# cc-ai/climategan

Hardware: AMD Instinct MI355X
Metric: 640x640 images/sec (G+D step): per-domain sample slots per second of the joint Masker+Painter training step (update_G + update_D), global batch 32 per domain (higher is better)
Workload: dtype bf16

## Files before the change

climategan_amd/csrc/conv3x3_lds.h:

```cpp
#pragma once
#include "cgan_common.h"

struct Conv3x3LdsArgs {
  const uint16_t* x;
  const u32x4* w;
  const float* bias;
  const uint16_t* res;
  uint16_t* y;
  int n, h, w_;
  int hi, wi;
  int pad, reflect;
  int hx, wx;
  int cin;
  int cin_s, cin_p, cout, cout_s, ctiles, ksteps;
  int in_ups, act, has_res, res_ups;
  float slope;
  int shuffle;
  int shuffle_w;
  int k, stride;
};

bool conv3x3_lds_applicable(const CganConvDesc* d);
int conv3x3_lds_launch(const Conv3x3LdsArgs& a, int dtype, hipStream_t s);
bool conv_smallcin_applicable(const CganConvDesc* d);
int conv_smallcin_launch(const Conv3x3LdsArgs& a, int dtype, hipStream_t s);
```

climategan_amd/csrc/conv3x3_lds.hip:

```cpp
#include "conv3x3_lds.h"

namespace {

constexpr int TW = 16, TH = 16, WAVES = 4, PT = TH / WAVES;
constexpr int HPW = TW + 2, HPH = TH + 2, HP = HPH * HPW;
constexpr int XDMA = (HP * 4 + 63) / 64;
constexpr int XBUF_BYTES = XDMA * 1024;
constexpr int MAX_NCT = 5;
CGAN_KNOB(int, g_lds_nct, 0);
CGAN_KNOB(int, g_c4_enabled, 1);

__device__ __forceinline__ int xq_addr(int q, int slot) { return q * 64 + ((slot ^ ((q >> 1) & 3)) << 4); }

__device__ __attribute__((aligned(16))) unsigned int g_zeros[64];

__device__ __forceinline__ void halo_coord(const Conv3x3LdsArgs& p, int& yy, int& xx) {
  if (p.reflect) {
    yy = yy < 0 ? -yy : yy;
    xx = xx < 0 ? -xx : xx;
    yy = yy >= p.hi ? 2 * p.hi - 2 - yy : yy;
    xx = xx >= p.wi ? 2 * p.wi - 2 - xx : xx;
  }
}

#define STAGE_BARRIER()                                            \
  do {                                                             \
    asm volatile("s_waitcnt vmcnt(0) lgkmcnt(0)" ::: "memory");    \
    __builtin_amdgcn_s_barrier();                                  \
    asm volatile("" ::: "memory");                                 \
  } while (0)

template <typename T, int NCT, bool RES = true>
__device__ __forceinline__ void conv3x3_epilogue(const Conv3x3LdsArgs& p, f32x4 (&acc)[NCT][PT], unsigned char* smem,
                                                 int n, int ty0, int tx0, int ct0, int wave, int j, int g) {
  if (p.shuffle) {
    const int a = g >> 1, b = g & 1;
#pragma unroll
    for (int t = 0; t < PT; ++t) {
      const int yy = ty0 + wave * PT + t, xx = tx0 + j;
      const int oy = 2 * yy + a, ox = 2 * xx + b;
      if (yy < p.h && xx < p.w_ && oy < p.shuffle && ox < p.shuffle_w && ct0 == 0) {
        const f32x4 v = acc[0][t];
        const u32x4 o = {pack2<T>(v[0], v[1]), pack2<T>(v[2], v[3]), 0u, 0u};
        *reinterpret_cast<u32x4*>(p.y + (((size_t)n * p.shuffle + oy) * p.shuffle_w + ox) * 8) = o;
      }
    }
    return;
  }
  __syncthreads();
  unsigned char* yt = smem;
  const bool pad_c = p.cout < p.cout_s;
  f32x4 bias_q[NCT];
#pragma unroll
  for (int c = 0; c < NCT; ++c) {
    const int ch = (ct0 + c) * 16 + g * 4;
    bias_q[c] = (p.bias && ch < p.cout_s) ? *reinterpret_cast<const f32x4*>(p.bias + ch) : (f32x4){0.f, 0.f, 0.f, 0.f};
  }
  u32x2 rq[RES ? PT : 1][RES ? NCT : 1];
  if (RES && p.has_res) {
#pragma unroll
    for (int t = 0; t < PT; ++t) {
      const int yy = ty0 + wave * PT + t, xx = tx0 + j;
      const bool pin = yy < p.h && xx < p.w_;
      size_t rbase = 0;
      if (pin) {
        if (p.res_ups) rbase = (((size_t)n * (p.h >> 1) + (yy >> 1)) * (p.w_ >> 1) + (xx >> 1)) * p.cout_s;
        else rbase = (((size_t)n * p.h + yy) * p.w_ + xx) * p.cout_s;
      }
#pragma unroll
      for (int c = 0; c < NCT; ++c) {
        const int ch = (ct0 + c) * 16 + g * 4;
        rq[t][c] = (u32x2){0u, 0u};
        if (pin && ch < p.cout_s) rq[t][c] = *reinterpret_cast<const u32x2*>(p.res + rbase + ch);
      }
    }
    __builtin_amdgcn_sched_barrier(0);
    __builtin_amdgcn_s_waitcnt(0x0F70);
  }
#pragma unroll
  for (int t = 0; t < PT; ++t) {
    const int row = wave * PT + t;
    const int yy = ty0 + row, xx = tx0 + j;
    const bool pin = yy < p.h && xx < p.w_;
#pragma unroll
    for (int c = 0; c < NCT; ++c) {
      const int ch = (ct0 + c) * 16 + g * 4;
      float v[4];
#pragma unroll
      for (int r = 0; r < 4; ++r) v[r] = acc[c][t][r];
      if (ch < p.cout_s) {
#pragma unroll
        for (int r = 0; r < 4; ++r) v[r] += bias_q[c][r];
        if (RES && p.has_res && pin) {
          const u32x2 rv = rq[RES ? t : 0][RES ? c : 0];
          float r0, r1, r2, r3;
          unpack2<T>(rv[0], r0, r1);
          unpack2<T>(rv[1], r2, r3);
          v[0] = cgan_res_apply(v[0], r0, p.has_res); v[1] = cgan_res_apply(v[1], r1, p.has_res);
          v[2] = cgan_res_apply(v[2], r2, p.has_res); v[3] = cgan_res_apply(v[3], r3, p.has_res);
        }
        act_apply_n(v, p.act, p.slope);
        if (pad_c) {
#pragma unroll
          for (int r = 0; r < 4; ++r)
            if (ch + r >= p.cout) v[r] = 0.f;
        }
      }
      u32x2 o;
      o[0] = pack2<T>(v[0], v[1]);
      o[1] = pack2<T>(v[2], v[3]);
      *reinterpret_cast<u32x2*>(yt + ((row * 16 + j) * NCT + c) * 32 + g * 8) = o;
    }
  }
  __syncthreads();
#pragma unroll
  for (int k = 0; k < 2 * NCT; ++k) {
    const int id = k * (WAVES * 64) + threadIdx.x;
    const int pix = id / (2 * NCT), cc = id - pix * (2 * NCT);
    const int yy = ty0 + (pix >> 4), xx = tx0 + (pix & 15);
    const int ch = ct0 * 16 + cc * 8;
    if (yy < p.h && xx < p.w_ && ch < p.cout_s)
      CGAN_ST_STREAM(*reinterpret_cast<const u32x4*>(yt + id * 16),
                     reinterpret_cast<u32x4*>(p.y + (((size_t)n * p.h + yy) * p.w_ + xx) * p.cout_s + ch));
  }
}

template <typename T, int NCT>
__global__ __launch_bounds__(WAVES * 64, 2) void conv3x3_lds_kernel(Conv3x3LdsArgs p) {
  const u32x4* zero_page = reinterpret_cast<const u32x4*>(g_zeros);
  constexpr int STAGE_BYTES = 3 * NCT * 1024;
  extern __shared__ __attribute__((aligned(16))) unsigned char smem[];
  unsigned char* xbuf = smem;
  unsigned char* wbuf = xbuf + 2 * XBUF_BYTES;

  const int lane = threadIdx.x & 63;
  const int wave = __builtin_amdgcn_readfirstlane(threadIdx.x >> 6);
  const int j = lane & 15;
  const int g = lane >> 4;

  const int tiles_x = (p.w_ + TW - 1) / TW, tiles_y = (p.h + TH - 1) / TH;
  int tile = blockIdx.x;
  const int txi = tile % tiles_x;
  tile /= tiles_x;
  const int tyi = tile % tiles_y;
  const int n = tile / tiles_y;
  const int ty0 = tyi * TH, tx0 = txi * TW;
  const int ct0 = blockIdx.y * NCT;
  const int nq = p.cin_p / 32;
  const int nstages = nq * 3;

  auto issue_x = [&](int q) {
    unsigned char* dst = xbuf + (q & 1) * XBUF_BYTES;
    for (int i = wave; i < XDMA; i += WAVES) {
      const int idx = i * 64 + lane;
      const int pix = idx >> 2, spos = idx & 3;
      const int slot = spos ^ ((pix >> 1) & 3);
      const int py = pix / HPW, px = pix - py * HPW;
      int yy = ty0 - p.pad + py, xx = tx0 - p.pad + px;
      halo_coord(p, yy, xx);
      const int ch = q * 32 + slot * 8;
      const u32x4* src = zero_page;
      if (pix < HP && yy >= 0 && yy < p.hi && xx >= 0 && xx < p.wi && ch < p.cin_s) {
        const int sy = p.in_ups ? (yy >> 1) : yy, sx = p.in_ups ? (xx >> 1) : xx;
        src = reinterpret_cast<const u32x4*>(p.x + (((size_t)n * p.hx + sy) * p.wx + sx) * p.cin_s + ch);
      }
      __builtin_amdgcn_global_load_lds((const __attribute__((address_space(1))) void*)src,
                                       (__attribute__((address_space(3))) void*)(dst + i * 1024), 16, 0, 0);
    }
  };
  auto issue_w = [&](int s) {
    const int q = s / 3, dx = s - q * 3;
    unsigned char* dst = wbuf + (s & 1) * STAGE_BYTES;
#pragma unroll
    for (int i0 = 0; i0 < 3 * NCT; i0 += WAVES) {
      const int i = i0 + wave;
      if (i < 3 * NCT) {
        const int dy = i / NCT, c = i - dy * NCT;
        const int ct = min(ct0 + c, p.ctiles - 1);
        const u32x4* src = p.w + ((size_t)ct * p.ksteps + (dy * 3 + dx) * nq + q) * 64 + lane;
        __builtin_amdgcn_global_load_lds((const __attribute__((address_space(1))) void*)src,
                                         (__attribute__((address_space(3))) void*)(dst + i * 1024), 16, 0, 0);
      }
    }
  };

  issue_x(0);
  issue_w(0);

  f32x4 acc[NCT][PT];
#pragma unroll
  for (int c = 0; c < NCT; ++c)
#pragma unroll
    for (int t = 0; t < PT; ++t) acc[c][t] = (f32x4){0.f, 0.f, 0.f, 0.f};

  for (int q = 0; q < nq; ++q) {
    const unsigned char* xb = xbuf + (q & 1) * XBUF_BYTES;
    for (int dx = 0; dx < 3; ++dx) {
      const int s = q * 3 + dx;
      STAGE_BARRIER();
      if (dx == 0 && q + 1 < nq) issue_x(q + 1);
      if (s + 1 < nstages) issue_w(s + 1);
      u32x4 bfr[PT + 2];
#pragma unroll
      for (int r = 0; r < PT + 2; ++r) {
        const int qq = (wave * PT + r) * HPW + (j + dx);
        bfr[r] = *reinterpret_cast<const u32x4*>(xb + xq_addr(qq, g));
      }
      const unsigned char* wb = wbuf + (s & 1) * STAGE_BYTES + lane * 16;
#pragma unroll
      for (int dy = 0; dy < 3; ++dy) {
        u32x4 a[NCT];
#pragma unroll
        for (int c = 0; c < NCT; ++c) a[c] = *reinterpret_cast<const u32x4*>(wb + (dy * NCT + c) * 1024);
#pragma unroll
        for (int c = 0; c < NCT; ++c)
#pragma unroll
          for (int t = 0; t < PT; ++t)
            acc[c][t] = mfma16(as_vec8<T>(a[c]), as_vec8<T>(bfr[t + dy]), acc[c][t]);
      }
    }
  }

  conv3x3_epilogue<T, NCT>(p, acc, smem, n, ty0, tx0, ct0, wave, j, g);
}

template <typename T, int NCT>
__global__ __launch_bounds__(WAVES * 64, 4) void conv3x3_lds_onechunk_kernel(Conv3x3LdsArgs p) {
  const u32x4* zero_page = reinterpret_cast<const u32x4*>(g_zeros);
  extern __shared__ __attribute__((aligned(16))) unsigned char smem[];
  unsigned char* xbuf = smem;
  unsigned char* wbuf = xbuf + XBUF_BYTES;

  const int lane = threadIdx.x & 63;
  const int wave = __builtin_amdgcn_readfirstlane(threadIdx.x >> 6);
  const int j = lane & 15;
  const int g = lane >> 4;
  const int tiles_x = (p.w_ + TW - 1) / TW, tiles_y = (p.h + TH - 1) / TH;
  int tile = blockIdx.x;
  const int txi = tile % tiles_x;
  tile /= tiles_x;
  const int tyi = tile % tiles_y;
  const int n = tile / tiles_y;
  const int ty0 = tyi * TH, tx0 = txi * TW;
  const int ct0 = blockIdx.y * NCT;

  for (int i = wave; i < XDMA; i += WAVES) {
    const int idx = i * 64 + lane;
    const int pix = idx >> 2, spos = idx & 3;
    const int slot = spos ^ ((pix >> 1) & 3);
    const int py = pix / HPW, px = pix - py * HPW;
    int yy = ty0 - p.pad + py, xx = tx0 - p.pad + px;
    halo_coord(p, yy, xx);
    const int ch = slot * 8;
    const u32x4* src = zero_page;
    if (pix < HP && yy >= 0 && yy < p.hi && xx >= 0 && xx < p.wi && ch < p.cin_s) {
      const int sy = p.in_ups ? (yy >> 1) : yy, sx = p.in_ups ? (xx >> 1) : xx;
      src = reinterpret_cast<const u32x4*>(p.x + (((size_t)n * p.hx + sy) * p.wx + sx) * p.cin_s + ch);
    }
    __builtin_amdgcn_global_load_lds((const __attribute__((address_space(1))) void*)src,
                                     (__attribute__((address_space(3))) void*)(xbuf + i * 1024), 16, 0, 0);
  }
#pragma unroll
  for (int i0 = 0; i0 < 9 * NCT; i0 += WAVES) {
    const int i = i0 + wave;
    if (i < 9 * NCT) {
      const int tap = i / NCT, c = i - tap * NCT;
      const int ct = min(ct0 + c, p.ctiles - 1);
      const u32x4* src = p.w + ((size_t)ct * p.ksteps + tap) * 64 + lane;
      __builtin_amdgcn_global_load_lds((const __attribute__((address_space(1))) void*)src,
                                       (__attribute__((address_space(3))) void*)(wbuf + i * 1024), 16, 0, 0);
    }
  }

  f32x4 acc[NCT][PT];
#pragma unroll
  for (int c = 0; c < NCT; ++c)
#pragma unroll
    for (int t = 0; t < PT; ++t) acc[c][t] = (f32x4){0.f, 0.f, 0.f, 0.f};

  STAGE_BARRIER();
#pragma unroll
  for (int dx = 0; dx < 3; ++dx) {
    u32x4 bfr[PT + 2];
#pragma unroll
    for (int r = 0; r < PT + 2; ++r) {
      const int qq = (wave * PT + r) * HPW + (j + dx);
      bfr[r] = *reinterpret_cast<const u32x4*>(xbuf + xq_addr(qq, g));
    }
#pragma unroll
    for (int dy = 0; dy < 3; ++dy) {
      u32x4 a[NCT];
#pragma unroll
      for (int c = 0; c < NCT; ++c)
        a[c] = *reinterpret_cast<const u32x4*>(wbuf + ((dy * 3 + dx) * NCT + c) * 1024 + lane * 16);
#pragma unroll
      for (int c = 0; c < NCT; ++c)
#pragma unroll
        for (int t = 0; t < PT; ++t)
          acc[c][t] = mfma16(as_vec8<T>(a[c]), as_vec8<T>(bfr[t + dy]), acc[c][t]);
    }
  }
  conv3x3_epilogue<T, NCT>(p, acc, smem, n, ty0, tx0, ct0, wave, j, g);
}

template <typename T, int NCT>
__global__ __launch_bounds__(WAVES * 64, NCT <= 2 ? 8 : (NCT <= 4 ? 4 : 2)) void conv3x3_c4_kernel(Conv3x3LdsArgs p) {
  extern __shared__ __attribute__((aligned(16))) unsigned char smem[];
  const int lane = threadIdx.x & 63;
  const int wave = __builtin_amdgcn_readfirstlane(threadIdx.x >> 6);
  const int j = lane & 15;
  const int g = lane >> 4;
  const int tiles_x = (p.w_ + TW - 1) / TW, tiles_y = (p.h + TH - 1) / TH;
  int tile = blockIdx.x;
  const int txi = tile % tiles_x;
  tile /= tiles_x;
  const int tyi = tile % tiles_y;
  const int n = tile / tiles_y;
  const int ty0 = tyi * TH, tx0 = txi * TW;
  const int ct0 = blockIdx.y * NCT;

  u32x2* xh = reinterpret_cast<u32x2*>(smem);
  for (int pix = threadIdx.x; pix < HP; pix += WAVES * 64) {
    const int py = pix / HPW, px = pix - py * HPW;
    int yy = ty0 - p.pad + py, xx = tx0 - p.pad + px;
    halo_coord(p, yy, xx);
    u32x2 v = {0u, 0u};
    if (yy >= 0 && yy < p.hi && xx >= 0 && xx < p.wi) {
      const int sy = p.in_ups ? (yy >> 1) : yy, sx = p.in_ups ? (xx >> 1) : xx;
      v = *reinterpret_cast<const u32x2*>(p.x + (((size_t)n * p.hx + sy) * p.wx + sx) * p.cin_s);
    }
    xh[pix] = v;
  }
  u32x4 a0[NCT], a1[NCT];
#pragma unroll
  for (int c = 0; c < NCT; ++c) {
    const int ct = min(ct0 + c, p.ctiles - 1);
    const u32x2* wt = reinterpret_cast<const u32x2*>(p.w + (size_t)ct * p.ksteps * 64);
    const u32x2 lo = wt[((2 * g) * 64 + j) * 2], hi = wt[((2 * g + 1) * 64 + j) * 2];
    const u32x2 last = wt[(8 * 64 + j) * 2];
    a0[c] = (u32x4){lo[0], lo[1], hi[0], hi[1]};
    a1[c] = g == 0 ? (u32x4){last[0], last[1], 0u, 0u} : (u32x4){0u, 0u, 0u, 0u};
  }
  f32x4 acc[NCT][PT];
#pragma unroll
  for (int c = 0; c < NCT; ++c)
#pragma unroll
    for (int t = 0; t < PT; ++t) acc[c][t] = (f32x4){0.f, 0.f, 0.f, 0.f};
  __syncthreads();

  const int tA = 2 * g, tB = 2 * g + 1;
  const int offA = (tA / 3) * HPW + tA % 3, offB = (tB / 3) * HPW + tB % 3;
#pragma unroll
  for (int t = 0; t < PT; ++t) {
    const int base = (wave * PT + t) * HPW + j;
    const u32x2 lo = xh[base + offA], hi = xh[base + offB];
    const u32x2 last = xh[base + 2 * HPW + 2];
    const u32x4 b0 = {lo[0], lo[1], hi[0], hi[1]};
    const u32x4 b1 = g == 0 ? (u32x4){last[0], last[1], 0u, 0u} : (u32x4){0u, 0u, 0u, 0u};
#pragma unroll
    for (int c = 0; c < NCT; ++c) {
      acc[c][t] = mfma16(as_vec8<T>(a0[c]), as_vec8<T>(b0), acc[c][t]);
      acc[c][t] = mfma16(as_vec8<T>(a1[c]), as_vec8<T>(b1), acc[c][t]);
    }
  }
  conv3x3_epilogue<T, NCT, false>(p, acc, smem, n, ty0, tx0, ct0, wave, j, g);
}

template <typename T, int NCT>
__global__ __launch_bounds__(WAVES * 64, 4) void conv_smallcin_kernel(Conv3x3LdsArgs p) {
  extern __shared__ __attribute__((aligned(16))) unsigned char smem[];
  const int lane = threadIdx.x & 63;
  const int wave = __builtin_amdgcn_readfirstlane(threadIdx.x >> 6);
  const int j = lane & 15;
  const int g = lane >> 4;
  const int tiles_x = (p.w_ + TW - 1) / TW, tiles_y = (p.h + TH - 1) / TH;
  int tile = blockIdx.x;
  const int txi = tile % tiles_x;
  tile /= tiles_x;
  const int tyi = tile % tiles_y;
  const int n = tile / tiles_y;
  const int ty0 = tyi * TH, tx0 = txi * TW;
  const int hp = (TW - 1) * p.stride + p.k;
  const int taps = p.k * p.k;

  u32x4* xh = reinterpret_cast<u32x4*>(smem);
  const int iy0 = ty0 * p.stride - p.pad, ix0 = tx0 * p.stride - p.pad;
  for (int pix = threadIdx.x; pix < hp * hp; pix += WAVES * 64) {
    const int py = pix / hp, px = pix - py * hp;
    const int yy = iy0 + py, xx = ix0 + px;
    u32x4 v = {0u, 0u, 0u, 0u};
    if (yy >= 0 && yy < p.hi && xx >= 0 && xx < p.wi)
      v = *reinterpret_cast<const u32x4*>(p.x + (((size_t)n * p.hi + yy) * p.wi + xx) * 8);
    xh[pix] = v;
  }
  f32x4 acc[NCT][PT];
#pragma unroll
  for (int c = 0; c < NCT; ++c)
#pragma unroll
    for (int t = 0; t < PT; ++t) acc[c][t] = (f32x4){0.f, 0.f, 0.f, 0.f};
  auto load_a = [&](int ks, u32x4 (&a)[NCT]) {
#pragma unroll
    for (int c = 0; c < NCT; ++c) {
      const int ct = min(c, p.ctiles - 1);
      a[c] = p.w[((size_t)ct * p.ksteps + ks) * 64 + lane];
    }
  };
  u32x4 a_cur[NCT], a_nxt[NCT];
  load_a(0, a_cur);
  __syncthreads();
  for (int ks = 0; ks < p.ksteps; ++ks) {
    if (ks + 1 < p.ksteps) load_a(ks + 1, a_nxt);
    const int tap = ks * 4 + g;
    const bool tv = tap < taps;
    const int tc = tv ? tap : 0;
    const int ky = tc / p.k, kx = tc - ky * p.k;
    u32x4 b[PT];
#pragma unroll
    for (int t = 0; t < PT; ++t) {
      const int row = wave * PT + t;
      b[t] = xh[(row * p.stride + ky) * hp + j * p.stride + kx];
      if (!tv) b[t] = (u32x4){0u, 0u, 0u, 0u};
    }
#pragma unroll
    for (int c = 0; c < NCT; ++c)
#pragma unroll
      for (int t = 0; t < PT; ++t) acc[c][t] = mfma16(as_vec8<T>(a_cur[c]), as_vec8<T>(b[t]), acc[c][t]);
#pragma unroll
    for (int c = 0; c < NCT; ++c) a_cur[c] = a_nxt[c];
  }
  conv3x3_epilogue<T, NCT, false>(p, acc, smem, n, ty0, tx0, 0, wave, j, g);
}

template <typename T, int NCT>
int launch_smallcin(const Conv3x3LdsArgs& a, hipStream_t s) {
  const int tiles = a.n * ((a.h + TH - 1) / TH) * ((a.w_ + TW - 1) / TW);
  const int hp = (TW - 1) * a.stride + a.k;
  size_t smem = (size_t)hp * hp * 16;
  const size_t epi = (size_t)256 * NCT * 32;
  if (epi > smem) smem = epi;
  hipLaunchKernelGGL((conv_smallcin_kernel<T, NCT>), dim3(tiles), dim3(WAVES * 64), smem, s, a);
  return CGAN_OK;
}

template <typename T>
int launch_smallcin_any(const Conv3x3LdsArgs& a, hipStream_t s) {
  switch (a.ctiles) {
    case 1: return launch_smallcin<T, 1>(a, s);
    case 2: return launch_smallcin<T, 2>(a, s);
    case 3: return launch_smallcin<T, 3>(a, s);
    default: return launch_smallcin<T, 4>(a, s);
  }
}

template <typename T, int NCT>
int launch_c4(const Conv3x3LdsArgs& a, hipStream_t s) {
  const int tiles = a.n * ((a.h + TH - 1) / TH) * ((a.w_ + TW - 1) / TW);
  const size_t smem = (size_t)256 * NCT * 32;
  static bool attr_set = false;
  if (!attr_set) {
    hipError_t e = hipFuncSetAttribute(reinterpret_cast<const void*>(&conv3x3_c4_kernel<T, NCT>),
                                       hipFuncAttributeMaxDynamicSharedMemorySize, 160 * 1024);
    if (e != hipSuccess) {
      cgan_set_error("conv3x3_c4: hipFuncSetAttribute failed: %s", hipGetErrorString(e));
      return CGAN_ERR_HIP;
    }
    attr_set = true;
  }
  hipLaunchKernelGGL((conv3x3_c4_kernel<T, NCT>), dim3(tiles, ceil_div(a.ctiles, NCT)), dim3(WAVES * 64), smem, s, a);
  return CGAN_OK;
}

template <typename T, int NCT>
int launch(const Conv3x3LdsArgs& a, hipStream_t s) {
  const int tiles = a.n * ((a.h + TH - 1) / TH) * ((a.w_ + TW - 1) / TW);
  const int chunks = ceil_div(a.ctiles, NCT);
  size_t smem = (size_t)2 * XBUF_BYTES + 2 * 3 * NCT * 1024;
  const size_t epi = (size_t)256 * NCT * 32;
  if (epi > smem) smem = epi;
  static bool attr_set = false;
  if (!attr_set) {
    hipError_t e = hipFuncSetAttribute(reinterpret_cast<const void*>(&conv3x3_lds_kernel<T, NCT>),
                                       hipFuncAttributeMaxDynamicSharedMemorySize, 160 * 1024);
    if (e != hipSuccess) {
      cgan_set_error("conv3x3_lds: hipFuncSetAttribute failed: %s", hipGetErrorString(e));
      return CGAN_ERR_HIP;
    }
    attr_set = true;
  }
  if (NCT <= 2 && a.cin_p == 32) {
    size_t smem1 = (size_t)XBUF_BYTES + 9 * NCT * 1024;
    if (epi > smem1) smem1 = epi;
    static bool attr1_set = false;
    if (!attr1_set) {
      hipError_t e = hipFuncSetAttribute(reinterpret_cast<const void*>(&conv3x3_lds_onechunk_kernel<T, (NCT <= 2 ? NCT : 1)>),
                                         hipFuncAttributeMaxDynamicSharedMemorySize, 160 * 1024);
      if (e != hipSuccess) {
        cgan_set_error("conv3x3_lds: hipFuncSetAttribute failed: %s", hipGetErrorString(e));
        return CGAN_ERR_HIP;
      }
      attr1_set = true;
    }
    hipLaunchKernelGGL((conv3x3_lds_onechunk_kernel<T, (NCT <= 2 ? NCT : 1)>), dim3(tiles, chunks), dim3(WAVES * 64), smem1,
                       s, a);
    return CGAN_OK;
  }
  hipLaunchKernelGGL((conv3x3_lds_kernel<T, NCT>), dim3(tiles, chunks), dim3(WAVES * 64), smem, s, a);
  return CGAN_OK;
}

template <typename T>
int launch_nct(const Conv3x3LdsArgs& a, hipStream_t s) {
  if (g_c4_enabled && a.cin <= 4 && a.cin_p == 32 && a.ksteps == 9 && (a.cin_s & 3) == 0 && !a.has_res) {
    const long wg4 = (long)a.n * ((a.h + TH - 1) / TH) * ((a.w_ + TW - 1) / TW) * ceil_div(a.ctiles, 4);
    if (a.ctiles <= 2 || g_c4_enabled == 3 || (g_c4_enabled == 1 && wg4 < 8192)) return launch_c4<T, 2>(a, s);
    if (a.ctiles <= 4 || g_c4_enabled != 2) return launch_c4<T, 4>(a, s);
    return launch_c4<T, 8>(a, s);
  }
  if (g_lds_nct >= 1 && g_lds_nct <= MAX_NCT) {
    switch (g_lds_nct) {
      case 1: return launch<T, 1>(a, s);
      case 2: return launch<T, 2>(a, s);
      case 3: return launch<T, 3>(a, s);
      case 4: return launch<T, 4>(a, s);
      default: return launch<T, 5>(a, s);
    }
  }
  int nct = a.ctiles < MAX_NCT ? a.ctiles : MAX_NCT;
  if (a.ctiles > MAX_NCT) {
    int best = MAX_NCT, waste = ceil_div(a.ctiles, MAX_NCT) * MAX_NCT - a.ctiles;
    for (int k = MAX_NCT - 1; k >= 3; --k) {
      int w = ceil_div(a.ctiles, k) * k - a.ctiles;
      if (w < waste) { waste = w; best = k; }
    }
    nct = best;
  }
  switch (nct) {
    case 1: return launch<T, 1>(a, s);
    case 2: return launch<T, 2>(a, s);
    case 3: return launch<T, 3>(a, s);
    case 4: return launch<T, 4>(a, s);
    default: return launch<T, 5>(a, s);
  }
}

}

CGAN_DEV_ONLY(extern "C" void cgan_debug_set_conv3x3_c4(int v) { g_c4_enabled = v; })
CGAN_DEV_ONLY(extern "C" void cgan_debug_set_conv3x3_nct(int v) { g_lds_nct = v; })

bool conv3x3_lds_applicable(const CganConvDesc* d) {
  const bool pad_ok = d->pad_mode == CGAN_PAD_ZERO ? (d->pad >= 0 && d->pad <= 2)
                                                   : (d->pad == 1 && d->h_in >= 2 && d->w_in >= 2 && !d->in_upsample);
  return d->kh == 3 && d->kw == 3 && d->stride == 1 && d->dilation == 1 && pad_ok && (long)d->h_out * d->w_out >= 1024;
}

bool conv_smallcin_applicable(const CganConvDesc* d) {
  const int cs = cgan_cs(d->c_in);
  return cs == 8 && d->kh == d->kw && d->kh != 3 && d->kh >= 2 && d->kh <= 7 && (d->stride == 1 || d->stride == 2) &&
         d->dilation == 1 && d->pad_mode == CGAN_PAD_ZERO && d->pad >= 0 && d->pad <= d->kh && !d->in_upsample &&
         cgan_cs(d->c_out) <= 64 && !d->has_residual && (long)d->h_out * d->w_out >= 1024 &&
         (double)d->n * d->h_in * d->w_in * 16.0 < 4294967295.0;
}

int conv_smallcin_launch(const Conv3x3LdsArgs& a, int dtype, hipStream_t s) {
  return dtype == CGAN_F16 ? launch_smallcin_any<F16>(a, s) : launch_smallcin_any<BF16>(a, s);
}

int conv3x3_lds_launch(const Conv3x3LdsArgs& a, int dtype, hipStream_t s) {
  return dtype == CGAN_F16 ? launch_nct<F16>(a, s) : launch_nct<BF16>(a, s);
}
```

climategan_amd/csrc/conv_mfma.hip:

```cpp
#include "cgan_common.h"
#include "conv3x3_lds.h"
#include "conv_gemm.h"

namespace {

struct ConvParams {
  const uint16_t* x;
  const u32x4* w;
  const float* bias;
  const uint16_t* res;
  const uint16_t* res2;
  uint16_t* y;
  int n, h_in, w_in, hx, wx, cin_s, cin_p, cg;
  int cout, cout_s, ctiles;
  int kh, kw, stride, pad, dil, pad_mode;
  int h_out, w_out, npix;
  int kgroups, ksteps;
  int in_ups, act, has_res, res_ups;
  int in_zs;
  int cls_s;
  int cls_pad;
  float slope;
  float* stats;
  int pair;
// ... 771 lines not shown
  a.stats = p.stats;
  return a;
}

Conv3x3LdsArgs lds_args(const ConvPlan& pl) {
  const ConvParams& p = pl.p;
  Conv3x3LdsArgs a;
  a.x = p.x; a.w = p.w; a.bias = p.bias; a.res = p.res; a.y = p.y;
  a.n = p.n; a.h = p.h_out; a.w_ = p.w_out; a.hi = p.h_in; a.wi = p.w_in; a.pad = p.pad;
  a.reflect = p.pad_mode == CGAN_PAD_REFLECT;
  a.hx = p.hx; a.wx = p.wx; a.cin = pl.d.c_in; a.cin_s = p.cin_s; a.cin_p = p.cin_p;
  a.cout = p.cout; a.cout_s = p.cout_s; a.ctiles = p.ctiles; a.ksteps = p.ksteps;
  a.in_ups = p.in_ups; a.act = p.act; a.has_res = p.has_res; a.res_ups = p.res_ups; a.slope = p.slope;
  a.shuffle = 0; a.shuffle_w = 0; a.k = 0; a.stride = 0;
  if (pl.route == ROUTE_SMALLCIN) {
    a.k = p.kh; a.stride = p.stride; a.res_ups = 0;
  } else if (pl.route == ROUTE_SUBPIXEL) {
    a.h = a.hi = p.hx; a.w_ = a.wi = p.wx; a.pad = 1; a.slope = 0.f;
    a.cout = 16; a.cout_s = 16; a.ctiles = 1; a.ksteps = 9 * (a.cin_p / 32);
    a.shuffle = p.h_out; a.shuffle_w = p.w_out;
  }
  return a;
}

void cls_table(const ConvParams& p, ConvGemmCls (&cls)[4]) {
  int koff = 0;
  for (int c = 0; c < p.cls_s * p.cls_s; ++c) {
    const int ca = c / p.cls_s, cb = c % p.cls_s;
    int ry, rx, nty, ntx;
    cls_axis(p.cls_s, p.kh, p.cls_pad, ca, ry, nty);
    cls_axis(p.cls_s, p.kw, p.cls_pad, cb, rx, ntx);
    cls[c] = ConvGemmCls{koff, nty, ntx, (ca - p.cls_pad + ry) / p.cls_s, (cb - p.cls_pad + rx) / p.cls_s};
    if (nty * ntx == 0) cls[c].kh = cls[c].kw = 0;
    koff += cls_ksteps(p.cls_s, p.kh, p.kw, p.cls_pad, p.cg, c);
  }
}

ConvRoute route_stride1(ConvPlan& pl, bool stats, const WsSlot& ws) {
  const ConvParams& p = pl.p;
  const CganConvDesc* d = &pl.d;
  const bool lds = conv3x3_lds_applicable(d);
  const bool prefer_3x3 = lds && p.cin_s < 256 && g_conv_force != 3;
  if ((g_conv_force == 0 || g_conv_force == 3) && !prefer_3x3 && conv_gemm_applicable(d)) return ROUTE_GEMM;
  ConvRoute r = ROUTE_GENERAL;
  if (g_conv_force != 1 && lds) r = ROUTE_LDS3X3;
  else if (g_conv_force == 0 && conv_smallcin_applicable(d)) r = ROUTE_SMALLCIN;
  if ((r == ROUTE_GENERAL || (r == ROUTE_LDS3X3 && p.cin_s >= 256)) && g_conv_force == 0 && !stats && !p.in_ups &&
      p.cin_p == p.cin_s) {
    const ConvGemmArgs a = gemm_args(p);
    const int ks = conv_gemm_splitk_plan(a);
    if (ks > 1 && conv_gemm_splitk_workspace_bytes(a, ks) <= ws.bytes) {
      pl.ksplit = ks;
      pl.ws = (float*)ws.ws;
      return ROUTE_SPLITK;
    }
  }
  return r;
}

int plan_fwd(ConvPlan& pl, const CganConvDesc* d, int mode, const WsSlot& ws) {
  ConvParams& p = pl.p;
  int rc = fill_params(p, d);
  if (rc != CGAN_OK) return rc;
  pl.d = *d; pl.ksplit = 1; pl.ws = nullptr;
  if (mode != FWD_PAIR) {
    pl.route = route_stride1(pl, mode == FWD_STATS, ws);
    return CGAN_OK;
  }
  const int nb = cgan_split_blocks(d->dtype), ns = cgan_split_store_blocks(d->dtype);
  CGAN_REQUIRE((d->c_in % (8 * nb)) == 0, "conv2d_nhwc_fwd_pair: c_in must be the %d * round_up(C, 8) storage channels of a split map", nb);
  CGAN_REQUIRE((double)p.npix * p.cout_s * ns * 2.0 < 4294967295.0, "conv2d_nhwc_fwd_pair: output map of 4 GiB or more");
  p.pair = 1;
  p.csb = p.cin_s / nb;
  p.xs = ns * p.csb;
  pl.route = ROUTE_GENERAL;
  if (g_conv_force == 0 && !p.in_ups && p.cin_p == p.cin_s && p.npix >= 1024 && p.ksteps >= 4) {
    const ConvGemmArgs a = gemm_args(p);
    if (g_pair_big && conv_gemm_big_pair_ok(a, d->dtype)) pl.route = ROUTE_PAIR_BIG;
    else if (conv_gemm_ext_shape_ok(a) && (double)p.npix * p.cout_s * ns < 2147483647.0) pl.route = ROUTE_PAIR_GEMM;
  }
  return CGAN_OK;
}

int plan_dgrad(ConvPlan& pl, const CganConvDesc* f, int res_mode, const WsSlot& ws) {
  ConvParams& p = pl.p;
  CganConvDesc& t = pl.d;
  int rc = dgrad_desc(f, &t);
  if (rc != CGAN_OK) return rc;
  const int pad_t = t.pad;
  if (pad_t < 0) {
    t.pad = 0;
    t.h_out = t.h_in; t.w_out = t.w_in;
  }
  rc = fill_params(p, &t);
  if (rc != CGAN_OK) return rc;
  pl.ksplit = 1; pl.ws = nullptr;
  t.pad = p.pad = pad_t;
  t.h_out = p.h_out = f->h_in; t.w_out = p.w_out = f->w_in;
  p.npix = f->n * f->h_in * f->w_in;
  p.hx = f->h_out; p.wx = f->w_out;
  p.in_zs = f->stride;
  if (f->stride > 1 && f->dilation == 1 && pad_t >= 0 && g_dgrad_zero_insert == 0) {
    p.cls_s = f->stride; p.cls_pad = pad_t; p.in_zs = 1;
    p.h_in = p.hx; p.w_in = p.wx;
  }
  const bool plain = f->stride == 1 && pad_t >= 0 && t.h_in + 2 * pad_t - t.dilation * (t.kh - 1) == t.h_out &&
                     t.w_in + 2 * pad_t - t.dilation * (t.kw - 1) == t.w_out;
  if (res_mode != RES_NONE) {
    CGAN_REQUIRE(plain, "conv2d_nhwc_bwd_data_add / _relu: only for stride-1 'same' convolutions");
    p.has_res = res_mode == RES_ADD_RELU ? RES_ADD : res_mode;
    p.res_ups = 0;
    t.has_residual = 1;
  }
  if (plain) {
    pl.route = route_stride1(pl, false, ws);
    if (res_mode == RES_ADD_RELU && pl.route == ROUTE_GEMM && conv_gemm_res2_ok(gemm_args(p), t.dtype)) p.has_res = 3;
  } else if (dgrad_subpixel(f)) {
    pl.route = ROUTE_SUBPIXEL;
  } else if (p.cls_s && p.cls_s <= 2 && g_conv_force == 0 && p.cin_p == p.cin_s && conv_gemm_ext_shape_ok(gemm_args(p)) &&
             p.cout_s >= 64) {
    pl.route = ROUTE_CLS_GEMM;
  } else {
    pl.route = ROUTE_GENERAL;
  }
  return CGAN_OK;
}

int route_family(ConvRoute r) {
  switch (r) {
    case ROUTE_GENERAL: return CGAN_CONV_KERNEL_GENERAL;
    case ROUTE_LDS3X3: case ROUTE_SMALLCIN: case ROUTE_SUBPIXEL: return CGAN_CONV_KERNEL_LDS3X3;
    default: return CGAN_CONV_KERNEL_GEMM;
  }
}

int stats_chunk_pixels(const ConvPlan& pl) {
  const CganConvDesc& d = pl.d;
  if (pl.route != ROUTE_GEMM || d.has_residual || d.act != CGAN_ACT_NONE || d.in_upsample) return 0;
  static const float bias_present = 0.f;
  ConvGemmArgs a = gemm_args(pl.p);
  a.bias = d.has_bias ? &bias_present : nullptr;
  return conv_gemm_stats_chunk_pixels(a, d.dtype);
}

int launch_plan(const ConvPlan& pl, hipStream_t s, const char* what) {
  const ConvParams& p = pl.p;
  const int dt = pl.d.dtype;
  int rc = CGAN_OK;
  switch (pl.route) {
    case ROUTE_GEMM: rc = conv_gemm_launch(gemm_args(p), dt, s); break;
    case ROUTE_SPLITK: rc = conv_gemm_splitk_launch(gemm_args(p), pl.ksplit, pl.ws, dt, s); break;
    case ROUTE_LDS3X3: case ROUTE_SUBPIXEL: rc = conv3x3_lds_launch(lds_args(pl), dt, s); break;
    case ROUTE_SMALLCIN: rc = conv_smallcin_launch(lds_args(pl), dt, s); break;
    case ROUTE_CLS_GEMM: {
      ConvGemmCls cls[4];
      cls_table(p, cls);
      rc = conv_gemm_cls_launch(gemm_args(p), p.cls_s, cls, dt, s);
      break;
    }
    case ROUTE_PAIR_BIG: rc = conv_gemm_big_pair_launch(gemm_args(p), dt, s); break;
    case ROUTE_PAIR_GEMM: rc = conv_gemm_pair_launch(gemm_args(p), dt, s); break;
    case ROUTE_GENERAL:
      if (dt == CGAN_F16) launch<F16>(p, s);
      else launch<BF16>(p, s);
      break;
  }
  if (rc != CGAN_OK) return rc;
  CGAN_CHECK_LAUNCH(what);
  return CGAN_OK;
}

void bind(ConvParams& p, const void* x, const void* w, const float* bias, const void* res, void* y) {
  p.x = (const uint16_t*)x; p.w = (const u32x4*)w; p.bias = bias; p.res = (const uint16_t*)res; p.y = (uint16_t*)y;
}
}

extern "C" int cgan_conv2d_nhwc_fwd(const void* x, const void* packed_w, const float* bias_padded, const void* residual,
                                    void* y, const CganConvDesc* d, void* stream) {
  CGAN_REQUIRE(x && packed_w && y, "conv2d_nhwc_fwd: null pointer");
  ConvPlan pl;
  int rc = plan_fwd(pl, d, FWD_PLAIN, ws_lookup(stream));
  if (rc != CGAN_OK) return rc;
  CGAN_REQUIRE(!d->has_bias || bias_padded, "conv2d_nhwc_fwd: has_bias but bias is null");
  CGAN_REQUIRE(!d->has_residual || residual, "conv2d_nhwc_fwd: has_residual but residual is null");
  bind(pl.p, x, packed_w, d->has_bias ? bias_padded : nullptr, residual, y);
  return launch_plan(pl, (hipStream_t)stream, "conv2d_nhwc_fwd");
}

extern "C" int cgan_conv2d_nhwc_fwd_pair(const void* x3, const void* packed_w3, const float* bias_padded,
                                         const void* residual3, void* y3, const CganConvDesc* d, void* stream) {
  CGAN_REQUIRE(x3 && packed_w3 && y3, "conv2d_nhwc_fwd_pair: null pointer");
  ConvPlan pl;
  int rc = plan_fwd(pl, d, FWD_PAIR, WsSlot{});
  if (rc != CGAN_OK) return rc;
  CGAN_REQUIRE(!d->has_bias || bias_padded, "conv2d_nhwc_fwd_pair: has_bias but bias is null");
  CGAN_REQUIRE(!d->has_residual || residual3, "conv2d_nhwc_fwd_pair: has_residual but residual is null");
  bind(pl.p, x3, packed_w3, d->has_bias ? bias_padded : nullptr, residual3, y3);
  return launch_plan(pl, (hipStream_t)stream, "conv2d_nhwc_fwd_pair");
}

extern "C" int32_t cgan_conv2d_stats_chunk_pixels(const CganConvDesc* d) {
  ConvPlan pl;
  if (plan_fwd(pl, d, FWD_STATS, WsSlot{}) != CGAN_OK) return 0;
  return stats_chunk_pixels(pl);
}

extern "C" int cgan_conv2d_nhwc_fwd_stats(const void* x, const void* packed_w, const float* bias_padded, void* y,
                                          float* partial, size_t partial_bytes, const CganConvDesc* d, void* stream) {
  CGAN_REQUIRE(x && packed_w && y && partial, "conv2d_nhwc_fwd_stats: null pointer");
  ConvPlan pl;
  int rc = plan_fwd(pl, d, FWD_STATS, WsSlot{});
  if (rc != CGAN_OK) return rc;
  CGAN_REQUIRE(!d->has_bias || bias_padded, "conv2d_nhwc_fwd_stats: has_bias but bias is null");
  const int ppb = stats_chunk_pixels(pl);
  CGAN_REQUIRE(ppb > 0, "conv2d_nhwc_fwd_stats: this descriptor's kernel writes no statistics "
                        "(cgan_conv2d_stats_chunk_pixels returned 0)");
  const size_t need = (size_t)(pl.p.npix / ppb) * pl.p.cout_s * 2 * sizeof(float);
  if (partial_bytes < need) {
    cgan_set_error("conv2d_nhwc_fwd_stats: partial buffer %zu B < required %zu B", partial_bytes, need);
    return CGAN_ERR_WORKSPACE;
  }
  bind(pl.p, x, packed_w, d->has_bias ? bias_padded : nullptr, nullptr, y);
  pl.p.stats = partial;
  return launch_plan(pl, (hipStream_t)stream, "conv2d_nhwc_fwd_stats");
}

static size_t dgrad_packed_fragments(const ConvParams& p) {
  if (!p.cls_s) return (size_t)p.ctiles * p.ksteps * 64;
  size_t ks = 0;
  for (int c = 0; c < p.cls_s * p.cls_s; ++c) ks += cls_ksteps(p.cls_s, p.kh, p.kw, p.cls_pad, p.cg, c);
  return (size_t)p.ctiles * ks * 64;
}

extern "C" size_t cgan_conv2d_dgrad_packed_weight_bytes(const CganConvDesc* fwd) {
  ConvPlan pl;
  if (plan_dgrad(pl, fwd, RES_NONE, WsSlot{}) != CGAN_OK) return 0;
  if (pl.route == ROUTE_SUBPIXEL) {
    const Conv3x3LdsArgs a = lds_args(pl);
    return (size_t)a.ctiles * a.ksteps * 64 * 16;
  }
  const size_t fr = dgrad_packed_fragments(pl.p);
  return (fr ? fr : 64) * 16;
}

extern "C" int cgan_conv2d_pack_weight_dgrad(const float* w_oihw, const float* sigma, void* packed,
                                             const CganConvDesc* fwd, void* stream) {
  ConvPlan pl;
  int rc = plan_dgrad(pl, fwd, RES_NONE, WsSlot{});
  if (rc != CGAN_OK) return rc;
  CGAN_REQUIRE(w_oihw && packed, "conv2d_pack_weight_dgrad: null pointer");
  const ConvParams& p = pl.p;
  const CganConvDesc& t = pl.d;
  hipStream_t s = (hipStream_t)stream;
  if (pl.route == ROUTE_SUBPIXEL) {
    const int cin_p = lds_args(pl).cin_p;
    const int tot = 9 * (cin_p / 32) * 64;
    if (fwd->dtype == CGAN_F16)
      hipLaunchKernelGGL(pack_dgrad_subpixel_kernel<F16>, dim3(ceil_div(tot, 256)), dim3(256), 0, s, w_oihw, sigma,
                         (uint16_t*)packed, fwd->c_out, fwd->c_in, cin_p);
    else
      hipLaunchKernelGGL(pack_dgrad_subpixel_kernel<BF16>, dim3(ceil_div(tot, 256)), dim3(256), 0, s, w_oihw, sigma,
                         (uint16_t*)packed, fwd->c_out, fwd->c_in, cin_p);
  } else if (p.cls_s) {
    int max_ks = 1;
    for (int c = 0; c < p.cls_s * p.cls_s; ++c) {
      const int k = cls_ksteps(p.cls_s, p.kh, p.kw, p.cls_pad, p.cg, c);
      max_ks = k > max_ks ? k : max_ks;
    }
    const int tot = p.ctiles * max_ks * 64;
    const dim3 grid(ceil_div(tot, 256) < 1024 ? ceil_div(tot, 256) : 1024, p.cls_s * p.cls_s);
    if (fwd->dtype == CGAN_F16)
      hipLaunchKernelGGL(pack_dgrad_classes_kernel<F16>, grid, dim3(256), 0, s, w_oihw, sigma, (uint16_t*)packed, t.c_out,
                         t.c_in, p.cin_p, t.kh, t.kw, p.ctiles, p.cls_s, p.cls_pad);
    else
      hipLaunchKernelGGL(pack_dgrad_classes_kernel<BF16>, grid, dim3(256), 0, s, w_oihw, sigma, (uint16_t*)packed, t.c_out,
                         t.c_in, p.cin_p, t.kh, t.kw, p.ctiles, p.cls_s, p.cls_pad);
  } else {
    const int total = p.ctiles * p.ksteps * 64;
    const int blocks = ceil_div(total, 256) < 2048 ? ceil_div(total, 256) : 2048;
    if (fwd->dtype == CGAN_F16)
      hipLaunchKernelGGL(pack_conv_weight_kernel<F16>, dim3(blocks), dim3(256), 0, s, w_oihw, (const float*)nullptr, sigma,
                         (uint16_t*)packed, (float*)nullptr, t.c_out, t.c_in, p.cin_p, t.kh, t.kw, p.ctiles, p.ksteps, 1);
    else
      hipLaunchKernelGGL(pack_conv_weight_kernel<BF16>, dim3(blocks), dim3(256), 0, s, w_oihw, (const float*)nullptr, sigma,
                         (uint16_t*)packed, (float*)nullptr, t.c_out, t.c_in, p.cin_p, t.kh, t.kw, p.ctiles, p.ksteps, 1);
  }
  CGAN_CHECK_LAUNCH("conv2d_pack_weight_dgrad");
  return CGAN_OK;
}

static int kernel_kind_impl(const CganConvDesc* d, int32_t bwd_data, const WsSlot& ws) {
  ConvPlan pl;
  const int rc = bwd_data ? plan_dgrad(pl, d, RES_NONE, ws) : plan_fwd(pl, d, FWD_PLAIN, ws);
  return rc != CGAN_OK ? rc : route_family(pl.route);
}

extern "C" int cgan_conv2d_kernel_kind_on(const CganConvDesc* d, int32_t bwd_data, void* stream) {
  return kernel_kind_impl(d, bwd_data, ws_lookup(stream));
}
extern "C" int cgan_conv2d_kernel_kind(const CganConvDesc* d, int32_t bwd_data) {
  return kernel_kind_impl(d, bwd_data, WsSlot{0, nullptr, nullptr, ws_max_bytes()});
}

static int bwd_data_impl(const void* dy, const void* packed_w_dgrad, const void* res, const void* relu_out, void* dx,
                         const CganConvDesc* fwd, void* stream, int res_mode) {
  CGAN_REQUIRE(dy && packed_w_dgrad && dx, "conv2d_nhwc_bwd_data: null pointer");
  ConvPlan pl;
  int rc = plan_dgrad(pl, fwd, res_mode, ws_lookup(stream));
  if (rc != CGAN_OK) return rc;
  bind(pl.p, dy, packed_w_dgrad, nullptr, res, dx);
  if (pl.p.has_res == 3) pl.p.res2 = (const uint16_t*)relu_out;
  rc = launch_plan(pl, (hipStream_t)stream, "conv2d_nhwc_bwd_data");
  if (rc != CGAN_OK || res_mode != RES_ADD_RELU || pl.p.has_res == 3) return rc;
  return cgan_act_bwd(relu_out, dx, dx, fwd->dtype, CGAN_ACT_RELU, 0.f,
                      (int64_t)fwd->n * fwd->h_in * fwd->w_in * cgan_cs(fwd->c_in), stream);
}

extern "C" int cgan_conv2d_nhwc_bwd_data(const void* dy, const void* packed_w_dgrad, void* dx, const CganConvDesc* fwd,
                                         void* stream) {
  return bwd_data_impl(dy, packed_w_dgrad, nullptr, nullptr, dx, fwd, stream, RES_NONE);
}

extern "C" int cgan_conv2d_nhwc_bwd_data_relu(const void* dy, const void* packed_w_dgrad, const void* relu_out, void* dx,
                                              const CganConvDesc* fwd, void* stream) {
  CGAN_REQUIRE(relu_out != nullptr, "conv2d_nhwc_bwd_data_relu: null pointer");
  return bwd_data_impl(dy, packed_w_dgrad, relu_out, nullptr, dx, fwd, stream, RES_RELU);
}

extern "C" int cgan_conv2d_nhwc_bwd_data_add_relu(const void* dy, const void* packed_w_dgrad, const void* dx_add,
                                                  const void* relu_out, void* dx, const CganConvDesc* fwd, void* stream) {
  CGAN_REQUIRE(dx_add != nullptr && relu_out != nullptr, "conv2d_nhwc_bwd_data_add_relu: null pointer");
  return bwd_data_impl(dy, packed_w_dgrad, dx_add, relu_out, dx, fwd, stream, RES_ADD_RELU);
}

extern "C" int cgan_conv2d_nhwc_bwd_data_add(const void* dy, const void* packed_w_dgrad, const void* dx_add, void* dx,
                                             const CganConvDesc* fwd, void* stream) {
  CGAN_REQUIRE(dx_add != nullptr, "conv2d_nhwc_bwd_data_add: null pointer");
  return bwd_data_impl(dy, packed_w_dgrad, dx_add, nullptr, dx, fwd, stream, RES_ADD);
}
```

Baseline: 58.50.

## Add persistent 3x3 conv kernel that keeps weights in LDS and double-buffers halos

Adds a persistent conv3x3 walk kernel, taken by default for small channel classes (cin 64 with two output tiles, or cin 32 with three) when there are many tiles. It launches one 8-wave workgroup per CU that loads all weights and bias into LDS once, then walks a contiguous range of tiles. The next tile's halo is DMA-prefetched into a second buffer while the current tile computes. The aim is to stop reloading weights for every tile and to overlap global loads with MFMA work, at the cost of large LDS use, lower occupancy and fixed CU-count grid sizing.

```diff
diff --git a/climategan_amd/csrc/conv3x3_lds.h b/climategan_amd/csrc/conv3x3_lds.h
--- a/climategan_amd/csrc/conv3x3_lds.h
+++ b/climategan_amd/csrc/conv3x3_lds.h
@@ -22,5 +22,6 @@
 
 bool conv3x3_lds_applicable(const CganConvDesc* d);
 int conv3x3_lds_launch(const Conv3x3LdsArgs& a, int dtype, hipStream_t s);
+bool conv3x3_lds_walks(const Conv3x3LdsArgs& a);
 bool conv_smallcin_applicable(const CganConvDesc* d);
 int conv_smallcin_launch(const Conv3x3LdsArgs& a, int dtype, hipStream_t s);
diff --git a/climategan_amd/csrc/conv3x3_lds.hip b/climategan_amd/csrc/conv3x3_lds.hip
--- a/climategan_amd/csrc/conv3x3_lds.hip
+++ b/climategan_amd/csrc/conv3x3_lds.hip
@@ -9,6 +9,8 @@
 constexpr int MAX_NCT = 5;
 CGAN_KNOB(int, g_lds_nct, 0);
 CGAN_KNOB(int, g_c4_enabled, 1);
+CGAN_KNOB(int, g_lds_walk, 0);
+CGAN_KNOB(int, g_lds_walk_max_wgs, 0);
 
 __device__ __forceinline__ int xq_addr(int q, int slot) { return q * 64 + ((slot ^ ((q >> 1) & 3)) << 4); }
 
@@ -30,14 +32,15 @@
     asm volatile("" ::: "memory");                                 \
   } while (0)
 
-template <typename T, int NCT, bool RES = true>
-__device__ __forceinline__ void conv3x3_epilogue(const Conv3x3LdsArgs& p, f32x4 (&acc)[NCT][PT], unsigned char* smem,
-                                                 int n, int ty0, int tx0, int ct0, int wave, int j, int g) {
+template <typename T, int NCT, bool RES = true, int PTT = PT, bool LDSB = false>
+__device__ __forceinline__ void conv3x3_epilogue(const Conv3x3LdsArgs& p, f32x4 (&acc)[NCT][PTT], unsigned char* smem,
+                                                 int n, int ty0, int tx0, int ct0, int wave, int j, int g,
+                                                 const float* bias_lds = nullptr) {
   if (p.shuffle) {
     const int a = g >> 1, b = g & 1;
 #pragma unroll
-    for (int t = 0; t < PT; ++t) {
-      const int yy = ty0 + wave * PT + t, xx = tx0 + j;
+    for (int t = 0; t < PTT; ++t) {
+      const int yy = ty0 + wave * PTT + t, xx = tx0 + j;
       const int oy = 2 * yy + a, ox = 2 * xx + b;
       if (yy < p.h && xx < p.w_ && oy < p.shuffle && ox < p.shuffle_w && ct0 == 0) {
         const f32x4 v = acc[0][t];
@@ -54,13 +57,14 @@
 #pragma unroll
   for (int c = 0; c < NCT; ++c) {
     const int ch = (ct0 + c) * 16 + g * 4;
-    bias_q[c] = (p.bias && ch < p.cout_s) ? *reinterpret_cast<const f32x4*>(p.bias + ch) : (f32x4){0.f, 0.f, 0.f, 0.f};
-  }
-  u32x2 rq[RES ? PT : 1][RES ? NCT : 1];
+    if (LDSB) bias_q[c] = *(const __attribute__((address_space(3))) f32x4*)(bias_lds + ch);
+    else bias_q[c] = (p.bias && ch < p.cout_s) ? *reinterpret_cast<const f32x4*>(p.bias + ch) : (f32x4){0.f, 0.f, 0.f, 0.f};
+  }
+  u32x2 rq[RES ? PTT : 1][RES ? NCT : 1];
   if (RES && p.has_res) {
 #pragma unroll
-    for (int t = 0; t < PT; ++t) {
-      const int yy = ty0 + wave * PT + t, xx = tx0 + j;
+    for (int t = 0; t < PTT; ++t) {
+      const int yy = ty0 + wave * PTT + t, xx = tx0 + j;
       const bool pin = yy < p.h && xx < p.w_;
       size_t rbase = 0;
       if (pin) {
@@ -78,8 +82,8 @@
     __builtin_amdgcn_s_waitcnt(0x0F70);
   }
 #pragma unroll
-  for (int t = 0; t < PT; ++t) {
-    const int row = wave * PT + t;
+  for (int t = 0; t < PTT; ++t) {
+    const int row = wave * PTT + t;
     const int yy = ty0 + row, xx = tx0 + j;
     const bool pin = yy < p.h && xx < p.w_;
 #pragma unroll
@@ -114,8 +118,8 @@
   }
   __syncthreads();
 #pragma unroll
-  for (int k = 0; k < 2 * NCT; ++k) {
-    const int id = k * (WAVES * 64) + threadIdx.x;
+  for (int k = 0; k < NCT * PTT / 2; ++k) {
+    const int id = k * (TH / PTT * 64) + threadIdx.x;
     const int pix = id / (2 * NCT), cc = id - pix * (2 * NCT);
     const int yy = ty0 + (pix >> 4), xx = tx0 + (pix & 15);
     const int ch = ct0 * 16 + cc * 8;
@@ -301,6 +305,125 @@
     }
   }
   conv3x3_epilogue<T, NCT>(p, acc, smem, n, ty0, tx0, ct0, wave, j, g);
+}
+
+__device__ __forceinline__ void walk_dma16(const void* src, const unsigned char* lds_dst) {
+  const unsigned lds = __builtin_amdgcn_readfirstlane(
+      (unsigned)reinterpret_cast<size_t>((__attribute__((address_space(3))) const unsigned char*)lds_dst));
+  unsigned keep;
+  asm volatile("s_mov_b32 %0, m0\n\ts_mov_b32 m0, %2\n\ts_nop 0\n\tglobal_load_lds_dwordx4 %1, off\n\ts_mov_b32 m0, %0"
+               : "=&s"(keep)
+               : "v"(src), "s"(lds)
+               : "memory");
+}
+
+template <int NQ, int NCT>
+constexpr int walk_xb() { return NQ * XBUF_BYTES > 256 * NCT * 32 ? NQ * XBUF_BYTES : 256 * NCT * 32; }
+template <int NQ, int NCT>
+constexpr int walk_smem() { return 9 * NQ * NCT * 1024 + 2 * walk_xb<NQ, NCT>() + NCT * 64; }
+
+constexpr int WALK_WAVES = 8;
+
+template <typename T, int NQ, int NCT>
+__global__ __launch_bounds__(WALK_WAVES * 64, 2) void conv3x3_walk_kernel(Conv3x3LdsArgs p, int tiles) {
+  constexpr int WV = WALK_WAVES, PTW = TH / WV;
+  constexpr int XB = walk_xb<NQ, NCT>();
+  const u32x4* zero_page = reinterpret_cast<const u32x4*>(g_zeros);
+  extern __shared__ __attribute__((aligned(16))) unsigned char smem[];
+  unsigned char* wbuf = smem;
+  unsigned char* xbuf = smem + 9 * NQ * NCT * 1024;
+  float* bias_lds = reinterpret_cast<float*>(xbuf + 2 * XB);
+
+  const int lane = threadIdx.x & 63;
+  const int wave = __builtin_amdgcn_readfirstlane(threadIdx.x >> 6);
+  const int j = lane & 15;
+  const int g = lane >> 4;
+  const int tiles_x = (p.w_ + TW - 1) / TW, tiles_y = (p.h + TH - 1) / TH;
+  const int t0 = (int)((long)tiles * blockIdx.x / gridDim.x), t1 = (int)((long)tiles * (blockIdx.x + 1) / gridDim.x);
+  if (t0 >= t1) return;
+
+  auto tile_origin = [&](int tile, int& n, int& ty0, int& tx0) {
+    const int txi = tile % tiles_x;
+    tile /= tiles_x;
+    const int tyi = tile % tiles_y;
+    n = tile / tiles_y;
+    ty0 = tyi * TH; tx0 = txi * TW;
+  };
+  auto issue_halo = [&](int tile, unsigned char* dst) {
+    int n, ty0, tx0;
+    tile_origin(tile, n, ty0, tx0);
+    for (int i = wave; i < XDMA; i += WV) {
+      const int idx = i * 64 + lane;
+      const int pix = idx >> 2, spos = idx & 3;
+      const int slot = spos ^ ((pix >> 1) & 3);
+      const int py = pix / HPW, px = pix - py * HPW;
+      int yy = ty0 - p.pad + py, xx = tx0 - p.pad + px;
+      halo_coord(p, yy, xx);
+      const bool in = pix < HP && yy >= 0 && yy < p.hi && xx >= 0 && xx < p.wi;
+      const int sy = p.in_ups ? (yy >> 1) : yy, sx = p.in_ups ? (xx >> 1) : xx;
+      const uint16_t* px0 = p.x + (((size_t)n * p.hx + sy) * p.wx + sx) * p.cin_s;
+#pragma unroll
+      for (int q = 0; q < NQ; ++q) {
+        const int ch = q * 32 + slot * 8;
+        const u32x4* src = (in && ch < p.cin_s) ? reinterpret_cast<const u32x4*>(px0 + ch) : zero_page;
+        walk_dma16(src, dst + q * XBUF_BYTES + i * 1024);
+      }
+    }
+  };
+
+  if (threadIdx.x < NCT * 16) bias_lds[threadIdx.x] = (p.bias && (int)threadIdx.x < p.cout_s) ? p.bias[threadIdx.x] : 0.f;
+  for (int i = wave; i < 9 * NQ * NCT; i += WV) {
+    const int s = i / (3 * NCT), r = i - s * (3 * NCT);
+    const int q = s / 3, dx = s - q * 3;
+    const int dy = r / NCT, c = r - dy * NCT;
+    const int ct = min(c, p.ctiles - 1);
+    const u32x4* src = p.w + ((size_t)ct * p.ksteps + (dy * 3 + dx) * NQ + q) * 64 + lane;
+    walk_dma16(src, wbuf + i * 1024);
+  }
+  issue_halo(t0, xbuf);
+  asm volatile("s_waitcnt vmcnt(0)" ::: "memory");
+
+  for (int tile = t0; tile < t1; ++tile) {
+    unsigned char* xb = xbuf + ((tile - t0) & 1) * XB;
+    asm volatile("s_waitcnt lgkmcnt(0)" ::: "memory");
+    __builtin_amdgcn_s_barrier();
+    asm volatile("" ::: "memory");
+    if (tile + 1 < t1) issue_halo(tile + 1, xbuf + ((tile + 1 - t0) & 1) * XB);
+
+    f32x4 acc[NCT][PTW];
+#pragma unroll
+    for (int c = 0; c < NCT; ++c)
+#pragma unroll
+      for (int t = 0; t < PTW; ++t) acc[c][t] = (f32x4){0.f, 0.f, 0.f, 0.f};
+#pragma unroll
+    for (int q = 0; q < NQ; ++q) {
+#pragma unroll
+      for (int dx = 0; dx < 3; ++dx) {
+        u32x4 bfr[PTW + 2];
+#pragma unroll
+        for (int r = 0; r < PTW + 2; ++r) {
+          const int qq = (wave * PTW + r) * HPW + (j + dx);
+          bfr[r] = *reinterpret_cast<const u32x4*>(xb + q * XBUF_BYTES + xq_addr(qq, g));
+        }
+        const unsigned char* wb = wbuf + (q * 3 + dx) * (3 * NCT * 1024) + lane * 16;
+#pragma unroll
+        for (int dy = 0; dy < 3; ++dy) {
+          u32x4 a[NCT];
+#pragma unroll
+          for (int c = 0; c < NCT; ++c) a[c] = *reinterpret_cast<const u32x4*>(wb + (dy * NCT + c) * 1024);
+#pragma unroll
+          for (int c = 0; c < NCT; ++c)
+#pragma unroll
+            for (int t = 0; t < PTW; ++t)
+              acc[c][t] = mfma16(as_vec8<T>(a[c]), as_vec8<T>(bfr[t + dy]), acc[c][t]);
+        }
+      }
+    }
+    asm volatile("s_waitcnt vmcnt(0)" ::: "memory");
+    int n, ty0, tx0;
+    tile_origin(tile, n, ty0, tx0);
+    conv3x3_epilogue<T, NCT, true, PTW, true>(p, acc, xb, n, ty0, tx0, 0, wave, j, g, bias_lds);
+  }
 }
 
 template <typename T, int NCT>
@@ -508,9 +631,67 @@
   return CGAN_OK;
 }
 
+bool takes_c4(const Conv3x3LdsArgs& a) {
+  return g_c4_enabled && a.cin <= 4 && a.cin_p == 32 && a.ksteps == 9 && (a.cin_s & 3) == 0 && !a.has_res;
+}
+
+constexpr int CUS = 256;
+constexpr int WALK_LDS = 160 * 1024;
+
+int walk_tiles(const Conv3x3LdsArgs& a) { return a.n * ((a.h + TH - 1) / TH) * ((a.w_ + TW - 1) / TW); }
+
+bool walk_fits(const Conv3x3LdsArgs& a) {
+  return !a.shuffle && !takes_c4(a) && a.ctiles >= 1 && a.ctiles <= 4 && (a.cin_p == 32 || a.cin_p == 64) &&
+         a.ksteps == 9 * (a.cin_p / 32);
+}
+
+int walk_grid(const Conv3x3LdsArgs& a) {
+  int grid = CUS;
+  if (g_lds_walk_max_wgs > 0) grid = g_lds_walk_max_wgs;
+  const int tiles = walk_tiles(a);
+  return grid < tiles ? grid : tiles;
+}
+
+bool walk_taken(const Conv3x3LdsArgs& a) {
+  if (g_lds_walk == 1 || !walk_fits(a)) return false;
+  if (g_lds_walk == 2) return true;
+  const int nq = a.cin_p / 32;
+  const bool cls = (nq == 2 && a.ctiles == 2) || (nq == 1 && a.ctiles == 3);
+  return cls && walk_tiles(a) >= 32 * walk_grid(a);
+}
+
+template <typename T, int NQ, int NCT>
+int launch_walk_inst(const Conv3x3LdsArgs& a, hipStream_t s) {
+  constexpr int smem = walk_smem<NQ, NCT>();
+  static_assert(smem <= WALK_LDS, "conv3x3_walk: LDS");
+  static bool attr_set = false;
+  if (!attr_set) {
+    hipError_t e = hipFuncSetAttribute(reinterpret_cast<const void*>(&conv3x3_walk_kernel<T, NQ, NCT>),
+                                       hipFuncAttributeMaxDynamicSharedMemorySize, WALK_LDS);
+    if (e != hipSuccess) {
+      cgan_set_error("conv3x3_walk: hipFuncSetAttribute failed: %s", hipGetErrorString(e));
+      return CGAN_ERR_HIP;
+    }
+    attr_set = true;
+  }
+  hipLaunchKernelGGL((conv3x3_walk_kernel<T, NQ, NCT>), dim3(walk_grid(a)), dim3(WALK_WAVES * 64), smem, s, a, walk_tiles(a));
+  return CGAN_OK;
+}
+
+template <typename T, int NQ>
+int launch_walk_nq(const Conv3x3LdsArgs& a, hipStream_t s) {
+  switch (a.ctiles) {
+    case 1: return launch_walk_inst<T, NQ, 1>(a, s);
+    case 2: return launch_walk_inst<T, NQ, 2>(a, s);
+    case 3: return launch_walk_inst<T, NQ, 3>(a, s);
+    default: return launch_walk_inst<T, NQ, 4>(a, s);
+  }
+}
+
 template <typename T>
 int launch_nct(const Conv3x3LdsArgs& a, hipStream_t s) {
-  if (g_c4_enabled && a.cin <= 4 && a.cin_p == 32 && a.ksteps == 9 && (a.cin_s & 3) == 0 && !a.has_res) {
+  if (walk_taken(a)) return a.cin_p == 32 ? launch_walk_nq<T, 1>(a, s) : launch_walk_nq<T, 2>(a, s);
+  if (takes_c4(a)) {
     const long wg4 = (long)a.n * ((a.h + TH - 1) / TH) * ((a.w_ + TW - 1) / TW) * ceil_div(a.ctiles, 4);
     if (a.ctiles <= 2 || g_c4_enabled == 3 || (g_c4_enabled == 1 && wg4 < 8192)) return launch_c4<T, 2>(a, s);
     if (a.ctiles <= 4 || g_c4_enabled != 2) return launch_c4<T, 4>(a, s);
@@ -547,6 +728,9 @@
 
 CGAN_DEV_ONLY(extern "C" void cgan_debug_set_conv3x3_c4(int v) { g_c4_enabled = v; })
 CGAN_DEV_ONLY(extern "C" void cgan_debug_set_conv3x3_nct(int v) { g_lds_nct = v; })
+CGAN_DEV_ONLY(extern "C" void cgan_debug_set_conv3x3_walk(int mode, int max_wgs) { g_lds_walk = mode; g_lds_walk_max_wgs = max_wgs; })
+
+bool conv3x3_lds_walks(const Conv3x3LdsArgs& a) { return walk_taken(a); }
 
 bool conv3x3_lds_applicable(const CganConvDesc* d) {
   const bool pad_ok = d->pad_mode == CGAN_PAD_ZERO ? (d->pad >= 0 && d->pad <= 2)
diff --git a/climategan_amd/csrc/conv_mfma.hip b/climategan_amd/csrc/conv_mfma.hip
--- a/climategan_amd/csrc/conv_mfma.hip
+++ b/climategan_amd/csrc/conv_mfma.hip
@@ -1097,6 +1097,16 @@
   return kernel_kind_impl(d, bwd_data, WsSlot{0, nullptr, nullptr, ws_max_bytes()});
 }
 
+#ifdef CGAN_DEV
+extern "C" int cgan_debug_conv3x3_walk_taken(const CganConvDesc* d, int32_t bwd_data) {
+  ConvPlan pl;
+  const WsSlot ws{0, nullptr, nullptr, ws_max_bytes()};
+  const int rc = bwd_data ? plan_dgrad(pl, d, RES_NONE, ws) : plan_fwd(pl, d, FWD_PLAIN, ws);
+  if (rc != CGAN_OK) return rc;
+  return pl.route == ROUTE_LDS3X3 && conv3x3_lds_walks(lds_args(pl)) ? 1 : 0;
+}
+#endif
+
 static int bwd_data_impl(const void* dy, const void* packed_w_dgrad, const void* res, const void* relu_out, void* dx,
                          const CganConvDesc* fwd, void* stream, int res_mode) {
   CGAN_REQUIRE(dy && packed_w_dgrad && dx, "conv2d_nhwc_bwd_data: null pointer");
```

Result: no change. 58.13 (-0.6%).
